# luicalrob/Triangulation-in-Deformable-Scenes

Measured on AMD Instinct MI355X. Metric: LM iterations/sec + ms/iter at 100k corr × 2 views; 1/2/4/8-GPU scaling, higher is better.
Workload: dtype f64

## Files before the change

### triangulation-in-deformable-scenes_amd/csrc/spcg.hip

```cpp
#include <hip/hip_runtime.h>

#include <algorithm>
#include <cstdio>
#include <type_traits>

#include "spcg.h"
#include "ticket.h"
#include "wave.h"

namespace deftri {
namespace sp {

using wv::wave_sum;
using wv::wave_max;

__device__ __forceinline__ double block_sum(double v, double *red4) {
    const int lane = threadIdx.x & 63, w = threadIdx.x >> 6;
    v = wave_sum(v);
    if (lane == 0) red4[w] = v;
    __syncthreads();
    const double s = (red4[0] + red4[1]) + (red4[2] + red4[3]);
    __syncthreads();
    return s;
}

__device__ __forceinline__ double pval(const double2 *__restrict__ zp, double beta, int64_t i) {
    const double2 v = zp[i];
    return __fma_rn(beta, v.y, v.x);
}

__device__ __forceinline__ int it_state(const SpDev &G, int it, double &beta) {
    beta = 0.0;
    if (G.rec[0] != 0.0) return (int)G.rec[0];
    const double *rk = G.red + (int64_t)kSpRed * it;
    if (rk[2] != 0.0) return (int)rk[2];
    if (rk[1] <= G.tol2 * G.red[1]) return kSpConverged;
    if (it >= G.max_it) return kSpBudget;
    if (it > 0) beta = rk[0] / G.red[(int64_t)kSpRed * (it - 1)];
    return 0;
}

__device__ __forceinline__ void record_stop(const SpDev &G, int it, int st) {
    if (G.rec[0] == 0.0) {
        G.rec[0] = st;
        G.rec[1] = it;
    }
}

__host__ __device__ __forceinline__ int row_grid(int nrb) { return 8 * ((max(nrb, 1) + 7) / 8); }
__device__ __forceinline__ int row_block(int b, int nrb) {
    const int seg = (max(nrb, 1) + 7) / 8;
    return (b & 7) * seg + (b >> 3);
}

__device__ __forceinline__ int heavy_dof(const SpDev &G, int h) { return h < G.Q ? 6 * h : 6 * G.Q + (h - G.Q); }

__device__ __forceinline__ bool gated_off(const int *g) { return g && !*g; }
__device__ __forceinline__ double lam_of(const SpDev &G, double lam) { return G.lam_dev ? *G.lam_dev : lam; }

__device__ __forceinline__ void publish(double *p, double v) { st_sc1(p, v); }
__device__ __forceinline__ double fetch(const double *p) {
    return ld_sc1(p);
}

__device__ __forceinline__ int tri3(int a, int b) { return a * (a + 1) / 2 + b; }
__device__ __forceinline__ int tri6(int a, int b) { return a * (a + 1) / 2 + b; }

template <class JT, int GU>
__global__ void __launch_bounds__(256) __attribute__((amdgpu_waves_per_eu(GU == 4 ? 5 : GU == 6 ? 4 : 1, GU == 4 ? 5 : GU == 6 ? 4 : 3)))
k_sp_glin_rows(const SpDev G, JT *__restrict__ pj) {
    __shared__ double red4[4];
    if (gated_off(G.lgate)) return;
    const int lb = row_block(blockIdx.x, G.nrb2);
    const int w = lb * 4 + (threadIdx.x >> 6), lane = threadIdx.x & 63;
    double mx = 0.0;
    if (w < G.nwaves) {
        const int l = G.rowmap[64 * w + lane];
        double D[6] = {0, 0, 0, 0, 0, 0}, bb[3] = {0, 0, 0};
        if (l >= 0) {
            for (int j = G.rep_off[l]; j < G.rep_off[l + 1]; j++) {
                const double *J = G.Jr + 6 * (int64_t)j;
                const double wt = G.Wr[j];
#pragma unroll
                for (int r = 0; r < 2; r++) {
                    const double er = G.Er[2 * (int64_t)j + r];
#pragma unroll
                    for (int a = 0; a < 3; a++) {
                        const double ja = J[3 * r + a] * wt;
#pragma unroll
                        for (int c = 0; c <= a; c++) D[tri3(a, c)] += ja * J[3 * r + c];
                        bb[a] -= J[3 * r + a] * (wt * er);
                    }
                }
            }
            const int d0 = G.dep_off[l], d1 = G.dep_off[l + 1];
            for (int jb = d0; jb < d1; jb += 4) {
                double Jb[4][4], wb[4], eb[4];
#pragma unroll
                for (int u = 0; u < 4; u++) {
                    const int64_t j = jb + u < d1 ? jb + u : jb;
#pragma unroll
                    for (int c = 0; c < 4; c++) Jb[u][c] = G.Jd[4 * j + c];
                    wb[u] = G.Wd[j];
                    eb[u] = G.Ed[j];
                }
#pragma unroll
                for (int u = 0; u < 4; u++) {
                    if (jb + u >= d1) break;
                    const int64_t j = jb + u;
                    const double *J = Jb[u];
                    const double wt = wb[u], er = eb[u];
#pragma unroll
                    for (int a = 0; a < 3; a++) {
                        const double ja = J[a] * wt;
#pragma unroll
                        for (int c = 0; c <= a; c++) D[tri3(a, c)] += ja * J[c];
                        bb[a] -= J[a] * (wt * er);
                        G.cdep[3 * j + a] = ja * J[3];
                    }
                    G.wss[j] = (J[3] * wt) * J[3];
                }
            }
        }
        double H[6];
#pragma unroll
        for (int k = 0; k < 6; k++) H[k] = D[k];
        const int64_t n = G.nslots * 64;
        struct Raw { double j0, j1, j2, w, x; };
        const double *__restrict__ Ja = G.Ja, *__restrict__ Wa = G.Wa, *__restrict__ Ea = G.Ea;
        const double *__restrict__ Jd = G.Jd, *__restrict__ Wd = G.Wd;
        const int64_t jld = G.jld;
        const bool w1 = G.Q == 1 && G.pinfo != nullptr;
        auto load = [&](int m) -> Raw {
            const bool dep = m <= -2;
            const int mm = max(m, 0), jj = max(-2 - m, 0);
            const double *pa = Ja + (int64_t)(3 * (mm & 3)) * jld + (mm >> 2);
            const double *pd = Jd + 4 * (int64_t)jj;
            const double *Jc = dep ? pd : pa;
            const int64_t st = dep ? 1 : jld;
            const double *W = dep ? Wd + jj : w1 ? G.pinfo : Wa + (mm >> 2);
            const double *X = dep ? pd + 3 : Ea + (mm >> 2);
            return Raw{Jc[0], Jc[st], Jc[2 * st], *W, *X};
        };
        auto value = [&](int m, const Raw &r, double *v, double &wt, double &er) {
            const bool arap = m >= 0, dep = m <= -2;
            v[0] = dep ? (r.j0 * r.w) * r.x : arap ? r.j0 : 0.0;
            v[1] = dep ? (r.j1 * r.w) * r.x : arap ? r.j1 : 0.0;
            v[2] = dep ? (r.j2 * r.w) * r.x : arap ? r.j2 : 0.0;
            wt = arap ? r.w : 0.0;
            er = arap ? r.x : 0.0;
        };
        auto add = [&](const double *v, double wt, double er) {
#pragma unroll
            for (int a = 0; a < 3; a++) {
                const double ja = v[a] * wt;
#pragma unroll
                for (int c = 0; c <= a; c++) H[tri3(a, c)] += ja * v[c];
                bb[a] -= v[a] * (wt * er);
            }
        };
        int64_t k = G.woff[w] * 64 + lane;
        const int64_t k1 = G.woff[w + 1] * 64 + lane;
        auto step = [&](auto U_, bool clamp) {
            constexpr int U = decltype(U_)::value;
            int m[U];
            int64_t kk[U];
            bool in[U];
            Raw r[U];
#pragma unroll
            for (int u = 0; u < U; u++) {
                in[u] = !clamp || k + 64 * u < k1;
                kk[u] = in[u] ? k + 64 * u : k1 - 64;
            }
#pragma unroll
            for (int u = 0; u < U; u++) m[u] = G.pmap[kk[u]];
#pragma unroll
            for (int u = 0; u < U; u++) r[u] = load(m[u]);
#pragma unroll
            for (int u = 0; u < U; u++) {
                double v[3], wt, er;
                value(m[u], r[u], v, wt, er);
                if (!in[u]) wt = er = 0.0;
                add(v, wt, er);
                if (pj)
#pragma unroll
                    for (int a = 0; a < 3; a++) pj[a * n + kk[u]] = (JT)v[a];
            }
            k += U * 64;
        };
        using I4 = std::integral_constant<int, 4>;
        if constexpr (GU == 4) {
            while (k + 3 * 64 < k1) step(I4{}, false);
        } else if constexpr (GU == 6) {
            while (k + 5 * 64 < k1) step(std::integral_constant<int, 6>{}, false);
            if (k + 4 * 64 < k1) step(std::integral_constant<int, 6>{}, true);
        } else {
            while (k + 7 * 64 < k1) step(std::integral_constant<int, 8>{}, false);
            if (k + 4 * 64 < k1) step(std::integral_constant<int, 8>{}, true);
        }
        if (k < k1) step(I4{}, true);
        if (G.wsplit[w]) {
#pragma unroll
            for (int k = 0; k < 6; k++) H[k] += __shfl_xor(H[k], 32);
#pragma unroll
            for (int a = 0; a < 3; a++) bb[a] += __shfl_xor(bb[a], 32);
        }
        if (l >= 0) {
#pragma unroll
            for (int k = 0; k < 6; k++) { G.Hv[6 * (int64_t)l + k] = H[k]; G.Dv[6 * (int64_t)l + k] = D[k]; }
            const int64_t o = G.hd + 3 * (int64_t)(G.row0 + l);
#pragma unroll
            for (int a = 0; a < 3; a++) G.b[o + a] = bb[a];
            mx = fmax(fabs(H[0]), fmax(fabs(H[2]), fabs(H[5])));
        }
    }
    mx = wave_max(mx);
    if ((threadIdx.x & 63) == 0) red4[threadIdx.x >> 6] = mx;
    __syncthreads();
    if (threadIdx.x == 0 && lb < max(G.nrb2, 1)) G.mpart[lb] = fmax(fmax(red4[0], red4[1]), fmax(red4[2], red4[3]));
}

__global__ void __launch_bounds__(256) k_sp_glin_blocks(const SpDev G) {
    __shared__ double red[kSpLin][4];
    if (gated_off(G.lgate)) return;
    const int2 gr = G.glb[blockIdx.x];
    const int4 d = G.blk[gr.x];
    const int kind = d.x & 0xff, owned = d.x >> 8;
    const int lane = threadIdx.x & 63, w = threadIdx.x >> 6;
    const int i = d.z + threadIdx.x;
    double *out = G.lpart + (int64_t)kSpLin * gr.x;
    if (kind == SP_ARAP) {
        if (!owned) return;
        double a[kSpLin];
#pragma unroll
        for (int k = 0; k < kSpLin; k++) a[k] = 0.0;
        const int iend = G.blk[gr.x + gr.y - 1].w;
        for (int ii = i; ii < iend; ii += 256) {
            double J[6];
#pragma unroll
            for (int r = 0; r < 6; r++) J[r] = G.Ja[(12 + r) * G.jld + ii];
            const double wv = G.Wa[ii], er = G.Ea[ii];
#pragma unroll
            for (int r = 0; r < 6; r++) {
                const double jr = J[r] * wv;
#pragma unroll
                for (int c = 0; c <= r; c++) a[tri6(r, c)] += jr * J[c];
                a[21 + r] -= J[r] * (wv * er);
            }
        }
        for (int k = threadIdx.x; k < kSpLin * (gr.y - 1); k += 256) out[kSpLin + k] = 0.0;
#pragma unroll
        for (int k = 0; k < kSpLin; k++) {
            const double v = wave_sum(a[k]);
            if (lane == 0) red[k][w] = v;
        }
        __syncthreads();
        if (threadIdx.x < kSpLin) {
            const int k = threadIdx.x;
            out[k] = (red[k][0] + red[k][1]) + (red[k][2] + red[k][3]);
        }
    } else {
        double h = 0.0, bs = 0.0;
        if (i < d.w) {
            const int le = G.dperm[i];
            const double js = G.Jd[4 * (int64_t)le + 3];
            h = G.wss[le];
            bs = -js * (G.Wd[le] * G.Ed[le]);
        }
        h = wave_sum(h);
        bs = wave_sum(bs);
        if (lane == 0) { red[0][w] = h; red[1][w] = bs; }
        __syncthreads();
        if (threadIdx.x < 2) {
            const int k = threadIdx.x;
            out[k] = (red[k][0] + red[k][1]) + (red[k][2] + red[k][3]);
        }
    }
}

__global__ void __launch_bounds__(256) k_sp_glin_heavy(const SpDev G) {
    __shared__ double lds[8][32];
    __shared__ int last;
    if (gated_off(G.lgate)) return;
    const int ch = blockIdx.x, h = G.ch_h[ch];
    const int dim = h < G.Q ? kSpLin : 2;
    const int c = threadIdx.x & 31, g = threadIdx.x >> 5;
    double acc = 0.0;
    if (c < dim) {
        int64_t k = G.ch_lo[ch] + g;
        const int64_t k1 = G.ch_lo[ch + 1];
        for (; k + 7 * 8 < k1; k += 64) {
            double v[8];
#pragma unroll
            for (int u = 0; u < 8; u++) v[u] = G.lpart[(int64_t)kSpLin * G.hv_blk[k + 8 * u] + c];
#pragma unroll
            for (int u = 0; u < 8; u++) acc += v[u];
        }
        for (; k < k1; k += 8) acc += G.lpart[(int64_t)kSpLin * G.hv_blk[k] + c];
    }
    lds[g][c] = acc;
    __syncthreads();
    if ((int)threadIdx.x < dim) {
        double t = 0.0;
#pragma unroll
        for (int gg = 0; gg < 8; gg++) t += lds[gg][threadIdx.x];
        publish(G.chpart + (int64_t)kSpLin * ch + threadIdx.x, t);
    }
    const int c0 = G.hch_off[h], c1 = G.hch_off[h + 1];
    if (threadIdx.x == 0) {
        __atomic_signal_fence(__ATOMIC_SEQ_CST);
        __builtin_amdgcn_s_waitcnt(0);
        __atomic_signal_fence(__ATOMIC_SEQ_CST);
        last = __hip_atomic_fetch_add(G.hcnt + h, 1, __ATOMIC_RELAXED, __HIP_MEMORY_SCOPE_AGENT) == c1 - c0 - 1;
    }
    __syncthreads();
    if (!last) return;
    acc = 0.0;
    if (c < dim)
        for (int j = c0 + g; j < c1; j += 8) acc += fetch(G.chpart + (int64_t)kSpLin * j + c);
    __syncthreads();
    lds[g][c] = acc;
    __syncthreads();
    if ((int)threadIdx.x < dim) {
        double t = 0.0;
#pragma unroll
        for (int gg = 0; gg < 8; gg++) t += lds[gg][threadIdx.x];
        const int q = threadIdx.x;
        if (h < G.Q) {
            if (q < 21) G.hl[21 * (int64_t)h + q] = t;
            else G.b[6 * (int64_t)h + q - 21] = t;
        } else {
            if (q == 0) G.hl[21 * (int64_t)G.Q + (h - G.Q)] = t;
            else G.b[6 * (int64_t)G.Q + (h - G.Q)] = t;
        }
    }
    if (threadIdx.x == 0) st_sc1(G.hcnt + h, 0);
}

__global__ void __launch_bounds__(256) k_sp_maxdiag(const SpDev G, double *out, int stage) {
    __shared__ double red4[4];
    if (gated_off(G.lgate)) return;
    double m = 0.0;
    if (stage == 0) {
        for (int i = threadIdx.x; i < G.nrb2; i += 256) m = fmax(m, G.mpart[i]);
    } else {
        for (int h = threadIdx.x; h < G.Q; h += 256)
#pragma unroll
            for (int a = 0; a < 6; a++) m = fmax(m, fabs(G.hl[21 * (int64_t)h + tri6(a, a)]));
        for (int s = threadIdx.x; s < G.S; s += 256) m = fmax(m, fabs(G.hl[21 * (int64_t)G.Q + s]));
    }
    m = wave_max(m);
    if ((threadIdx.x & 63) == 0) red4[threadIdx.x >> 6] = m;
    __syncthreads();
    if (threadIdx.x == 0) {
        const double v = fmax(fmax(red4[0], red4[1]), fmax(red4[2], red4[3]));
        out[0] = stage == 0 ? v : fmax(out[0], v);
    }
}

__global__ void k_sp_cvt_j(const double *__restrict__ J, float *__restrict__ J32, int64_t n, const int *gate) {
    if (gated_off(gate)) return;
    const int64_t i = (int64_t)blockIdx.x * 256 + threadIdx.x;
    if (i < n) J32[i] = (float)J[i];
}

__device__ __forceinline__ bool inv3(const double *A, double lam, double *M) {
    const double a00 = A[0] + lam, a10 = A[1], a11 = A[2] + lam, a20 = A[3], a21 = A[4], a22 = A[5] + lam;
    if (!(a00 > 0.0)) return false;
    const double l00 = sqrt(a00), l10 = a10 / l00, l20 = a20 / l00;
    const double d1 = a11 - l10 * l10;
    if (!(d1 > 0.0)) return false;
    const double l11 = sqrt(d1), l21 = (a21 - l20 * l10) / l11;
    const double d2 = a22 - l20 * l20 - l21 * l21;
    if (!(d2 > 0.0)) return false;
    const double l22 = sqrt(d2);
    const double i00 = 1.0 / l00, i11 = 1.0 / l11, i22 = 1.0 / l22;
    const double i10 = -l10 * i00 * i11;
    const double i21 = -l21 * i11 * i22;
    const double i20 = -(l20 * i00 + l21 * i10) * i22;
    M[0] = i00 * i00 + i10 * i10 + i20 * i20;
    M[1] = i11 * i10 + i21 * i20;
    M[2] = i11 * i11 + i21 * i21;
    M[3] = i22 * i20;
    M[4] = i22 * i21;
    M[5] = i22 * i22;
    return true;
}

__device__ __forceinline__ void mul3(const double *M, const double r[3], double z[3]) {
    z[0] = M[0] * r[0] + M[1] * r[1] + M[3] * r[2];
    z[1] = M[1] * r[0] + M[2] * r[1] + M[4] * r[2];
    z[2] = M[3] * r[0] + M[4] * r[1] + M[5] * r[2];
}

__device__ bool inv6(const double *Hl, double lam, double *Mo) {
    double L[36];
    for (int i = 0; i < 6; i++)
        for (int j = 0; j < 6; j++) L[i * 6 + j] = j <= i ? Hl[tri6(i, j)] + (i == j ? lam : 0.0) : 0.0;
    for (int j = 0; j < 6; j++) {
        double s = L[j * 6 + j];
        for (int k = 0; k < j; k++) s -= L[j * 6 + k] * L[j * 6 + k];
        if (!(s > 0.0)) return false;
        s = sqrt(s);
        L[j * 6 + j] = s;
        for (int i = j + 1; i < 6; i++) {
            double t = L[i * 6 + j];
            for (int k = 0; k < j; k++) t -= L[i * 6 + k] * L[j * 6 + k];
            L[i * 6 + j] = t / s;
        }
    }
    for (int c = 0; c < 6; c++) {
        double y[6];
        for (int i = 0; i < 6; i++) {
            double t = i == c ? 1.0 : 0.0;
            for (int k = 0; k < i; k++) t -= L[i * 6 + k] * y[k];
            y[i] = t / L[i * 6 + i];
        }
        for (int i = 5; i >= 0; i--) {
            double t = y[i];
            for (int k = i + 1; k < 6; k++) t -= L[k * 6 + i] * y[k];
            y[i] = t / L[i * 6 + i];
        }
        for (int i = 0; i < 6; i++) Mo[i * 6 + c] = y[i];
    }
    return true;
}

__device__ __forceinline__ void pair_tree(double a0, double a1, double (*red)[4], double *out, int pub = 0) {
    const int lane = threadIdx.x & 63, w = threadIdx.x >> 6;
    a0 = wave_sum(a0);
    a1 = wave_sum(a1);
    if (lane == 0) { red[0][w] = a0; red[1][w] = a1; }
    __syncthreads();
    if (threadIdx.x == 0) {
        const double s0 = (red[0][0] + red[0][1]) + (red[0][2] + red[0][3]);
        const double s1 = (red[1][0] + red[1][1]) + (red[1][2] + red[1][3]);
        if (pub == 1) {
            st_sc1(out, s0);
            st_sc1(out + 1, s1);
        } else {
            out[0] = s0;
            out[1] = s1;
        }
    }
}

__device__ __forceinline__ bool last_block(const SpDev &G, int *cnt) {
    __shared__ int last;
    if (threadIdx.x == 0) {
        __atomic_signal_fence(__ATOMIC_SEQ_CST);
        __builtin_amdgcn_s_waitcnt(0);
        __atomic_signal_fence(__ATOMIC_SEQ_CST);
        last = ticket_last(cnt, (int)gridDim.x, (int)blockIdx.x);
    }
    __syncthreads();
    return last;
}

template <int NV>
__device__ __forceinline__ bool group_sum(const SpDev &G, int *cnt, const double *slots, double *gs, double (*red)[4], double *tot) {
    __shared__ int flag;
    const int nb = (int)gridDim.x, x = (int)blockIdx.x & 7;
    const int gsize = (nb - x + 7) >> 3, ngroups = nb < 8 ? nb : 8;
    auto settle = [&] {
        __atomic_signal_fence(__ATOMIC_SEQ_CST);
        __builtin_amdgcn_s_waitcnt(0);
        __atomic_signal_fence(__ATOMIC_SEQ_CST);
    };
    if (threadIdx.x == 0) {
        settle();
        flag = __hip_atomic_fetch_add(cnt + 1 + x, 1, __ATOMIC_RELAXED, __HIP_MEMORY_SCOPE_AGENT) == gsize - 1;
    }
    __syncthreads();
    if (!flag) return false;
    double a[NV];
#pragma unroll
    for (int v = 0; v < NV; v++) a[v] = 0.0;
    for (int j = x + 8 * (int)threadIdx.x; j < nb; j += 8 * 256)
#pragma unroll
        for (int v = 0; v < NV; v++) a[v] += fetch(slots + NV * j + v);
    const int lane = threadIdx.x & 63, w = threadIdx.x >> 6;
#pragma unroll
    for (int v = 0; v < NV; v++) {
        a[v] = wave_sum(a[v]);
        if (lane == 0) red[v][w] = a[v];
    }
    __syncthreads();
    if (threadIdx.x == 0) {
#pragma unroll
        for (int v = 0; v < NV; v++) publish(gs + NV * x + v, (red[v][0] + red[v][1]) + (red[v][2] + red[v][3]));
        st_sc1(cnt + 1 + x, 0);
        settle();
        flag = __hip_atomic_fetch_add(cnt, 1, __ATOMIC_RELAXED, __HIP_MEMORY_SCOPE_AGENT) == ngroups - 1;
        if (flag) {
            st_sc1(cnt, 0);
#pragma unroll
            for (int v = 0; v < NV; v++) {
                double t = 0.0;
                for (int g = 0; g < ngroups; g++) t += fetch(gs + NV * g + v);
                tot[v] = t;
            }
        }
    }
    __syncthreads();
    return flag;
}

__device__ __forceinline__ void dots_block(const SpDev &G, int it, double (*red)[4]) {
    double a0 = 0.0, a1 = 0.0;
    int i = threadIdx.x;
    for (; i + 3 * 256 <= G.nrb; i += 4 * 256) {
        double v[4][2];
#pragma unroll
        for (int u = 0; u < 4; u++) { v[u][0] = fetch(G.upart + 2 * (i + 256 * u)); v[u][1] = fetch(G.upart + 2 * (i + 256 * u) + 1); }
#pragma unroll
        for (int u = 0; u < 4; u++) { a0 += v[u][0]; a1 += v[u][1]; }
    }
    for (; i <= G.nrb; i += 256) { a0 += fetch(G.upart + 2 * i); a1 += fetch(G.upart + 2 * i + 1); }
    pair_tree(a0, a1, red, G.red + (int64_t)kSpRed * it);
}

__device__ __forceinline__ void sd_send(const SpDev &G, int l, int a, double z, double p) {
    for (int k = G.snd_off[l]; k < G.snd_off[l + 1]; k++) {
        const int64_t o = 6 * (int64_t)G.snd_slot[k] + 2 * a;
        G.sbuf[o] = z;
        G.sbuf[o + 1] = p;
    }
}

__global__ void __launch_bounds__(3 * kSpUpdRows) k_sp_setup(const SpDev G, const double *__restrict__ rhs, double lam) {
    __shared__ double sM[6 * kSpUpdRows], sR[3 * kSpUpdRows];
    __shared__ double red[2][3 * kSpUpdRows / 64], dred[2][4];
    if (gated_off(G.gate)) return;
    lam = lam_of(G, lam);
    const int t = threadIdx.x, lane = t & 63, wv = t >> 6;
    constexpr int nw = 3 * kSpUpdRows / 64;
    double rz = 0.0, rr = 0.0;
    const int rb = (int)blockIdx.x - 1, slot = rb < 0 ? G.nrb : rb;
    if (rb < 0 && t < 32) st_sc1(G.cnt + t, 0);
    if (rb >= 0) {
        const int l0 = rb * kSpUpdRows;
        const int nrow = min(kSpUpdRows, G.nown - l0);
        const int64_t o0 = G.hd + 3 * (int64_t)(G.row0 + l0);
        const double *Hg = G.Hv + 6 * (int64_t)l0;
        if (t < 6 * nrow) sM[t] = Hg[t];
        if (t + 3 * kSpUpdRows < 6 * nrow) sM[t + 3 * kSpUpdRows] = Hg[t + 3 * kSpUpdRows];
        const double r = t < 3 * nrow ? rhs[o0 + t] : 0.0;
        sR[t] = r;
        __syncthreads();
        if (t < nrow) {
            double Hl[6], M[6];
#pragma unroll
            for (int k = 0; k < 6; k++) Hl[k] = sM[6 * t + k];
            if (!inv3(Hl, lam, M)) {
                G.rec[0] = kSpBadBlock;
#pragma unroll
                for (int k = 0; k < 6; k++) M[k] = 0.0;
            }
#pragma unroll
            for (int k = 0; k < 6; k++) sM[6 * t + k] = M[k];
        }
        __syncthreads();
        double *Mg = G.Mv + 6 * (int64_t)l0;
        if (t < 6 * nrow) Mg[t] = sM[t];
        if (t + 3 * kSpUpdRows < 6 * nrow) Mg[t + 3 * kSpUpdRows] = sM[t + 3 * kSpUpdRows];
        if (t < 3 * nrow) {
            const int row = t / 3, a = t - 3 * row;
            const double *M = sM + 6 * row;
            const int i0 = a == 0 ? 0 : a == 1 ? 1 : 3, i1 = a == 0 ? 1 : a == 1 ? 2 : 4, i2 = a == 0 ? 3 : a == 1 ? 4 : 5;
            const double *rv = sR + 3 * row;
            const double z = M[i0] * rv[0] + M[i1] * rv[1] + M[i2] * rv[2];
            G.r[o0 + t] = r;
            G.zp[o0 + t] = make_double2(z, 0.0);
            G.x[o0 + t] = 0.0;
            if (G.sd) sd_send(G, l0 + row, a, z, 0.0);
            rz = r * z;
            rr = r * r;
        }
    } else if (t < 256) {
        for (int h = t; h < G.Q + G.S; h += 256) {
// ... 1075 lines not shown
                    if (lane - d >= sstart) v[c] += y;
                }
            }
            if (valid && (m.x & kTmLast)) {
#pragma unroll
                for (int c = 0; c < 3; c++) { up[3 * ra + c] = v[c]; up[3 * rb + c] = v[3 + c]; }
            }
        }
        __syncthreads();
        if (tid < nr) {
            const int l = G.tmulti ? own_row(tid) : r0 + tid;
            const bool home = !G.tmulti || G.trow[r0 + tid] < 0;
            const int64_t o = G.hd + 3 * (int64_t)(G.row0 + l);
            double q[3], p[3];
#pragma unroll
            for (int c = 0; c < 3; c++) { q[c] = up[3 * tid + c]; p[c] = pL[3 * tid + c]; }
            const int sb = rsi & 0xffff, sc = rsi >> 16;
            for (int kk = sb; kk < sb + sc; kk++)
#pragma unroll
                for (int c = 0; c < 3; c++) q[c] += rs[3 * kk + c];
            if (home) {
                double D[6];
#pragma unroll
                for (int kk = 0; kk < 6; kk++) D[kk] = G.tmulti ? Dp[kk] : G.Dv[6 * (int64_t)l + kk];
                const double q0 = lam * p[0] + ((D[0] * p[0] + D[1] * p[1]) + D[3] * p[2]);
                const double q1 = lam * p[1] + ((D[1] * p[0] + D[2] * p[1]) + D[4] * p[2]);
                const double q2 = lam * p[2] + ((D[3] * p[0] + D[4] * p[1]) + D[5] * p[2]);
                pap += (p[0] * q0 + p[1] * q1) + p[2] * q2;
                q[0] += q0; q[1] += q1; q[2] += q2;
            }
            const int jend = G.tmulti ? (dsc0 >= 0 ? 1 : 0) : dj1 - dj0;
            for (int jj = 0; jj < jend; jj++) {
                const int j = dj0 + jj;
                const bool pre = G.tmulti != 0;
                const int sc_ = pre ? dsc0 : G.dsc[j];
                double cd[3];
#pragma unroll
                for (int c = 0; c < 3; c++) cd[c] = pre ? cd0[c] : G.cdep[3 * (int64_t)j + c];
                const double wsj = pre ? ws0 : G.wss[j];
                const double ps = hp[6 + sc_];
                const double cp = (cd[0] * p[0] + cd[1] * p[1]) + cd[2] * p[2];
                const double td = cp + wsj * ps;
                pap += ps * (cp + td);
                if (sc_ == 0) sacc[0] += td;
                else sacc[1] += td;
#pragma unroll
                for (int c = 0; c < 3; c++) q[c] += cd[c] * ps;
            }
            if (home) {
#pragma unroll
                for (int c = 0; c < 3; c++) G.q[o + c] = q[c];
            } else {
                const int64_t x = 3 * ((int64_t)(G.tdst[r0 + tid] - 1) * G.nown + l);
#pragma unroll
                for (int c = 0; c < 3; c++) G.qs[x + c] = q[c];
            }
        }
    }
    double a[9] = {pap, jts[0], jts[1], jts[2], jts[3], jts[4], jts[5], sacc[0], sacc[1]};
#pragma unroll
    for (int kk = 0; kk < 9; kk++) {
        const double v = wave_sum(a[kk]);
        if (lane == 0) red[kk][wv] = v;
    }
    __syncthreads();
    if (tid < 9) {
        const double v = (red[tid][0] + red[tid][1]) + (red[tid][2] + red[tid][3]);
        if (tid == 0) G.m1part[b] = v;
        else G.part[(int64_t)kSpPart * b + tid - 1] = v;
    }
}

template <int FIN>
__global__ void __launch_bounds__(256) k_sp_tupd(int it, const SpDev G, double lam, int last) {
    __shared__ double red4[4];
    if (gated_off(G.gate)) return;
    lam = lam_of(G, lam);
    double beta = 0.0;
    AlphaPre pf;
    const bool own_alpha = !FIN && !G.alpha_kernel && (G.tparts || blockIdx.x == 0);
    if (own_alpha) m2_alpha_loads(G, it, pf);
    if (const int st = it_state(G, it, beta)) {
        if (!FIN && blockIdx.x == 0 && threadIdx.x == 0) record_stop(G, it, st);
        return;
    }
    double alpha = 0.0, pq = 0.0, rr2 = 0.0;
    if (!FIN) {
        if (G.alpha_kernel) alpha = G.red[(int64_t)kSpRed * it + 3];
        else if (own_alpha) alpha = m2_alpha_make(G, it, red4, !G.tparts, pf, blockIdx.x == 0);
    }
    if ((int)blockIdx.x < G.m_nh) {
        __shared__ double lds[256];
        __shared__ double rsh[6], tz[2][6];
        const int h = blockIdx.x;
        const bool has = h < G.Q + G.S;
        const double th = has ? tile_heavy_sum(G, h, lds) : 0.0;
        if (!FIN && !own_alpha && !G.alpha_kernel) alpha = m2_alpha_wait(G, it);
        if (has) {
            const int dim = h < G.Q ? 6 : 1, o = heavy_dof(G, h);
            const int a = (!FIN && isnan(alpha)) ? dim : (int)threadIdx.x;
            double p = 0.0, r = 0.0;
            if (a < dim) {
                p = G.ph[o + a];
                const double q = th + lam * p;
                if (FIN) {
                    G.q[o + a] = q;
                } else {
                    G.x[o + a] += alpha * p;
                    r = G.r[o + a] - alpha * q;
                    G.r[o + a] = r;
                    rsh[a] = r;
                }
            }
            if (!FIN) {
                __syncthreads();
                if (a < dim) {
                    const double *Mh = h < G.Q ? G.Mh + 36 * (int64_t)h + a * 6 : G.Mh + 36 * (int64_t)G.Q + (h - G.Q);
                    double z = 0.0;
                    for (int c = 0; c < dim; c++) z += Mh[c] * rsh[c];
                    G.zp[o + a] = make_double2(z, p);
                    tz[0][a] = r * z;
                    tz[1][a] = r * r;
                }
                __syncthreads();
                if (threadIdx.x == 0 && !isnan(alpha))
                    for (int c = 0; c < dim; c++) { pq += tz[0][c]; rr2 += tz[1][c]; }
            }
        }
    } else {
        const int lb = row_block((int)blockIdx.x - G.m_nh, G.nrb);
        const int l = lb * 256 + (int)threadIdx.x;
        const bool on = l < G.nown;
        double q[3] = {0, 0, 0}, pr[3] = {0, 0, 0}, xo[3] = {0, 0, 0}, ro[3] = {0, 0, 0}, M[6] = {0, 0, 0, 0, 0, 0};
        int64_t o = 0;
        if (on) {
            o = G.hd + 3 * (int64_t)l;
#pragma unroll
            for (int c = 0; c < 3; c++) q[c] = G.q[o + c];
            if (G.tmulti) {
                const int ns = G.tnshare[l];
                for (int j0 = 1; j0 < ns; j0 += 4) {
                    double v[4][3];
#pragma unroll
                    for (int u = 0; u < 4; u++) {
                        const int j = j0 + u < ns ? j0 + u : j0;
                        const double *s = G.qs + 3 * ((int64_t)(j - 1) * G.nown + l);
#pragma unroll
                        for (int c = 0; c < 3; c++) v[u][c] = s[c];
                    }
#pragma unroll
                    for (int u = 0; u < 4; u++)
                        if (j0 + u < ns)
#pragma unroll
                            for (int c = 0; c < 3; c++) q[c] += v[u][c];
                }
            }
            {
                const int k0 = G.txoff[l], k1 = G.txoff[l + 1];
                for (int kb = k0; kb < k1; kb += 4) {
                    double v[4][3];
#pragma unroll
                    for (int u = 0; u < 4; u++) {
                        const int64_t k = kb + u < k1 ? kb + u : kb;
#pragma unroll
                        for (int c = 0; c < 3; c++) v[u][c] = G.xc[3 * k + c];
                    }
#pragma unroll
                    for (int u = 0; u < 4; u++)
                        if (kb + u < k1)
#pragma unroll
                            for (int c = 0; c < 3; c++) q[c] += v[u][c];
                }
            }
            if (FIN) {
#pragma unroll
                for (int c = 0; c < 3; c++) G.q[o + c] = q[c];
            } else {
#pragma unroll
                for (int c = 0; c < 3; c++) {
                    const double2 v = G.zp[o + c];
                    pr[c] = __fma_rn(beta, v.y, v.x);
                    xo[c] = G.x[o + c];
                    ro[c] = G.r[o + c];
                }
#pragma unroll
                for (int k = 0; k < 6; k++) M[k] = G.Mv[6 * (int64_t)l + k];
            }
        }
        if (!FIN && !own_alpha && !G.alpha_kernel) alpha = m2_alpha_wait(G, it);
        if (!FIN && on && !isnan(alpha)) {
            double r[3], z[3];
#pragma unroll
            for (int c = 0; c < 3; c++) {
                G.x[o + c] = xo[c] + alpha * pr[c];
                r[c] = ro[c] - alpha * q[c];
            }
            z[0] = M[0] * r[0] + M[1] * r[1] + M[3] * r[2];
            z[1] = M[1] * r[0] + M[2] * r[1] + M[4] * r[2];
            z[2] = M[3] * r[0] + M[4] * r[1] + M[5] * r[2];
#pragma unroll
            for (int c = 0; c < 3; c++) {
                G.r[o + c] = r[c];
                G.zp[o + c] = make_double2(z[c], pr[c]);
                pq += r[c] * z[c];
                rr2 += r[c] * r[c];
            }
        }
    }
    if (FIN) return;
    __shared__ double red[2][4];
    if (G.tparts && !last) {
        pair_tree(pq, rr2, red, G.m2part + 2 * blockIdx.x, 0);
        return;
    }
    pair_tree(pq, rr2, red, G.m2part + 2 * blockIdx.x, 1);
    m2_dots(G, it, red);
}

__global__ void __launch_bounds__(256) k_sp_txb(int it, const SpDev G) {
    __shared__ double red4[4];
    __shared__ double lds[256];
    (void)it;
    if (gated_off(G.gate) || G.rec[0] != 0.0) return;
    const int nh = G.Q + G.S, h = (int)blockIdx.x;
    if (h < nh) {
        const double t = tile_heavy_sum(G, h, lds);
        if ((int)threadIdx.x < (h < G.Q ? 6 : 1)) G.xb[3 + heavy_dof(G, h) + threadIdx.x] = t;
    } else if (h == nh) {
        double a = 0.0;
        for (int j = threadIdx.x; j < G.t_grid; j += 256) a += G.m1part[j];
        a = block_sum(a, red4);
        if (threadIdx.x == 0) G.xb[2] = a;
    } else {
        double a0 = 0.0, a1 = 0.0;
        for (int j = threadIdx.x; j <= G.nrb; j += 256) { a0 += G.upart[2 * j]; a1 += G.upart[2 * j + 1]; }
        a0 = block_sum(a0, red4);
        a1 = block_sum(a1, red4);
        if (threadIdx.x == 0) { G.xb[0] = a0; G.xb[1] = a1; }
    }
}


__global__ void k_sp_pack(int n, const int32_t *__restrict__ rows, int width, int64_t base, const double *__restrict__ src,
                          double *__restrict__ buf) {
    const int64_t t = (int64_t)blockIdx.x * 256 + threadIdx.x;
    if (t >= (int64_t)n * width) return;
    const int64_t i = t / width, c = t % width;
    buf[t] = src[base + (int64_t)width * rows[i] + c];
}

__global__ void k_sp_unpack(int n, const int32_t *__restrict__ rows, int width, int64_t base, const double *__restrict__ buf,
                            double *__restrict__ dst) {
    const int64_t t = (int64_t)blockIdx.x * 256 + threadIdx.x;
    if (t >= (int64_t)n * width) return;
    const int64_t i = t / width, c = t % width;
    dst[base + (int64_t)width * rows[i] + c] = buf[t];
}

__global__ void k_sp_load_p(int64_t n, const double *__restrict__ v, double2 *__restrict__ zp) {
    const int64_t t = (int64_t)blockIdx.x * 256 + threadIdx.x;
    if (t < n) zp[t] = make_double2(v[t], 0.0);
}

__global__ void k_sp_permute(int32_t P, int64_t hd, const int32_t *__restrict__ row_of_point, const double *__restrict__ src,
                             double *__restrict__ dst, int to_plan) {
    const int64_t t = (int64_t)blockIdx.x * 256 + threadIdx.x;
    if (t < hd) { dst[t] = src[t]; return; }
    const int64_t u = t - hd;
    if (u >= 3 * (int64_t)P) return;
    const int64_t pt = u / 3, c = u % 3;
    const int64_t row = row_of_point[pt];
    if (to_plan) dst[hd + 3 * row + c] = src[hd + 3 * pt + c];
    else dst[hd + 3 * pt + c] = src[hd + 3 * row + c];
}

}

static inline unsigned nblk(int64_t n, int bs) { return (unsigned)std::max<int64_t>((n + bs - 1) / bs, 1); }

#define SPL(NAME, KER, GRID, ...)                                          \
    do {                                                                   \
        if ((GRID) <= 0) break;                               \
        hipEvent_t e0_ = prof_begin(st);                                   \
        hipLaunchKernelGGL(KER, dim3(GRID), dim3(256), 0, st, __VA_ARGS__); \
        prof_end(NAME, e0_, (unsigned)(GRID), 0.0, st);                    \
    } while (0)

#define SPLS(NAME, KER, GRID, LDS, ...)                                              \
    do {                                                                             \
        if ((GRID) <= 0) break;                                                      \
        hipEvent_t e0_ = prof_begin(st);                                             \
        hipLaunchKernelGGL(KER, dim3(GRID), dim3(256), (size_t)(LDS), st, __VA_ARGS__); \
        prof_end(NAME, e0_, (unsigned)(GRID), 0.0, st);                              \
    } while (0)

template <class JT, int MG>
static void launch_phase2(const SpDev &G, int grid, int it, double lambda, const JT *pj, hipStream_t st) {
    if (G.p2u == 4) SPL("sp_phase2", (sp::k_sp_phase2<JT, MG, 4>), grid, it, G, lambda, pj);
    else if (G.p2u == 6) SPL("sp_phase2", (sp::k_sp_phase2<JT, MG, 6>), grid, it, G, lambda, pj);
    else SPL("sp_phase2", (sp::k_sp_phase2<JT, MG, 8>), grid, it, G, lambda, pj);
}

void sp_launch_glin(const SpDev &G, bool fp32, hipStream_t st) {
    if (G.glu == 4) {
        if (fp32) SPL("sp_glin_rows", (sp::k_sp_glin_rows<float, 4>), sp::row_grid(G.nrb2), G, G.pj32);
        else SPL("sp_glin_rows", (sp::k_sp_glin_rows<double, 4>), sp::row_grid(G.nrb2), G, G.pj);
    } else if (G.glu == 6) {
        if (fp32) SPL("sp_glin_rows", (sp::k_sp_glin_rows<float, 6>), sp::row_grid(G.nrb2), G, G.pj32);
        else SPL("sp_glin_rows", (sp::k_sp_glin_rows<double, 6>), sp::row_grid(G.nrb2), G, G.pj);
    } else {
        if (fp32) SPL("sp_glin_rows", (sp::k_sp_glin_rows<float, 8>), sp::row_grid(G.nrb2), G, G.pj32);
        else SPL("sp_glin_rows", (sp::k_sp_glin_rows<double, 8>), sp::row_grid(G.nrb2), G, G.pj);
    }
    if (G.nblk > 0) SPL("sp_glin_blocks", sp::k_sp_glin_blocks, G.nglb, G);
    if (G.nch > 0) SPL("sp_glin_heavy", sp::k_sp_glin_heavy, G.nch, G);
}

void sp_launch_maxdiag(const SpDev &G, double *out, hipStream_t st) {
    SPL("sp_maxdiag", sp::k_sp_maxdiag, 1, G, out, 0);
}

void sp_launch_maxdiag_heavy(const SpDev &G, double *out, hipStream_t st) {
    SPL("sp_maxdiag", sp::k_sp_maxdiag, 1, G, out, 1);
}

void sp_launch_cvt_j(const double *J, float *J32, int64_t n, hipStream_t st, const int *gate) {
    if (n > 0) SPL("sp_cvt_j", sp::k_sp_cvt_j, nblk(n, 256), J, J32, n, gate);
}

void sp_launch_setup(const SpDev &G, const double *rhs, double lambda, hipStream_t st) {
    const int grid = (G.nown + kSpUpdRows - 1) / kSpUpdRows + 1;
    hipEvent_t e0_ = prof_begin(st);
    hipLaunchKernelGGL(sp::k_sp_setup, dim3(grid), dim3(3 * kSpUpdRows), 0, st, G, rhs, lambda);
    prof_end("sp_setup", e0_, (unsigned)grid, 0.0, st);
}

void sp_launch_dots(const SpDev &G, int it, hipStream_t st) {
    SPL("sp_dots", sp::k_sp_dots, 1, it, G);
}

void sp_launch_product(const SpDev &G, int it, double lambda, bool fp32, hipStream_t st, bool last) {
    if (G.sd) {
        sp_launch_sd_phase1(G, it, lambda, fp32, st, nullptr, sp_merged_grid1(G));
        sp_launch_sd_phase2(G, it, lambda, fp32, st);
        return;
    }
    if (G.tile) {
        hipEvent_t e0_ = prof_begin(st);
        if (fp32) hipLaunchKernelGGL((sp::k_sp_tile<float>), dim3(G.t_grid), dim3(256), (size_t)G.tile_lds, st, it, G, G.Ja32, lambda);
        else hipLaunchKernelGGL((sp::k_sp_tile<double>), dim3(G.t_grid), dim3(256), (size_t)G.tile_lds, st, it, G, G.Ja, lambda);
        prof_end("sp_tile", e0_, (unsigned)G.t_grid, 0.0, st);
        if (G.alpha_kernel) SPL("sp_alpha", sp::k_sp_alpha, 1, it, G);
        SPL("sp_tupd", (sp::k_sp_tupd<0>), G.m_nh + sp::row_grid(G.nrb), it, G, lambda, last ? 1 : 0);
        return;
    }
    if (G.merged) {
        const int g1 = sp_merged_grid1(G), g2 = sp_merged_grid2(G);
        if (fp32) SPL("sp_phase1", (sp::k_sp_phase1<float, 1>), g1, it, G, G.Ja32, lambda);
        else SPL("sp_phase1", (sp::k_sp_phase1<double, 1>), g1, it, G, G.Ja, lambda);
        if (G.alpha_kernel) SPL("sp_alpha", sp::k_sp_alpha, 1, it, G);
        if (fp32) launch_phase2<float, 1>(G, g2, it, lambda, G.pj32, st);
        else launch_phase2<double, 1>(G, g2, it, lambda, G.pj, st);
        return;
    }
    if (G.nblk > 0) {
        if (fp32) SPL("sp_phase1", (sp::k_sp_phase1<float, 0>), G.nblk, it, G, G.Ja32, lambda);
        else SPL("sp_phase1", (sp::k_sp_phase1<double, 0>), G.nblk, it, G, G.Ja, lambda);
    }
    const int grid = sp::row_grid(G.nrb2) + (G.fuse_heavy ? G.Q + G.S : 0);
    if (fp32) launch_phase2<float, 0>(G, grid, it, lambda, G.pj32, st);
    else launch_phase2<double, 0>(G, grid, it, lambda, G.pj, st);
}

void sp_launch_tile_sd(const SpDev &G, int it, double lambda, bool fp32, hipStream_t st, const int32_t *list, int n,
                       bool txb) {
    if (n > 0) {
        SpDev g = G;
        g.p1list = list;
        hipEvent_t e0_ = prof_begin(st);
        if (fp32) hipLaunchKernelGGL((sp::k_sp_tile<float, 1>), dim3(n), dim3(256), (size_t)G.tile_lds, st, it, g, G.Ja32, lambda);
        else hipLaunchKernelGGL((sp::k_sp_tile<double, 1>), dim3(n), dim3(256), (size_t)G.tile_lds, st, it, g, G.Ja, lambda);
        prof_end("sp_tile", e0_, (unsigned)n, 0.0, st);
    }
    if (txb) SPL("sp_txb", sp::k_sp_txb, G.Q + G.S + 2, it, G);
}

void sp_launch_tile_product(const SpDev &G, double lambda, bool fp32, hipStream_t st) {
    hipEvent_t e0_ = prof_begin(st);
    if (fp32) hipLaunchKernelGGL((sp::k_sp_tile<float>), dim3(G.t_grid), dim3(256), (size_t)G.tile_lds, st, 0, G, G.Ja32, lambda);
    else hipLaunchKernelGGL((sp::k_sp_tile<double>), dim3(G.t_grid), dim3(256), (size_t)G.tile_lds, st, 0, G, G.Ja, lambda);
    prof_end("sp_tile", e0_, (unsigned)G.t_grid, 0.0, st);
    SPL("sp_tupd", (sp::k_sp_tupd<1>), G.m_nh + sp::row_grid(G.nrb), 0, G, lambda, 1);
}

int sp_merged_grid1(const SpDev &G) { return 8 * ((G.nrb + 1 + 7) / 8) + G.nblk; }

void sp_launch_sd_phase1(const SpDev &G, int it, double lambda, bool fp32, hipStream_t st, const int32_t *list, int n) {
    SpDev g = G;
    g.p1list = list;
    if (fp32) SPL("sp_phase1", (sp::k_sp_phase1<float, 2>), n, it, g, G.Ja32, lambda);
    else SPL("sp_phase1", (sp::k_sp_phase1<double, 2>), n, it, g, G.Ja, lambda);
}

void sp_launch_sd_phase2(const SpDev &G, int it, double lambda, bool fp32, hipStream_t st) {
    const int g2 = G.m_nh + sp::row_grid(G.nrb2);
    if (fp32) launch_phase2<float, 2>(G, g2, it, lambda, G.pj32, st);
    else launch_phase2<double, 2>(G, g2, it, lambda, G.pj, st);
}
int sp_merged_grid2(const SpDev &G) { return 8 * ((G.Q + G.S + 7) / 8) + sp::row_grid(G.nrb2); }

void sp_launch_heavy(const SpDev &G, int it, double lambda, int stage, hipStream_t st) {
    const int grid = (stage == 1 && G.heavy_split) ? G.Q + G.S + 1 : 1;
    SPL("sp_heavy", sp::k_sp_heavy, grid, it, G, lambda, stage);
}

void sp_launch_update_sd(const SpDev &G, int it, double lambda, int tail, hipStream_t st) {
    const int grid = (G.nown + kSpUpdRows - 1) / kSpUpdRows + 1;
    hipEvent_t e0_ = prof_begin(st);
    hipLaunchKernelGGL(sp::k_sp_update_sd, dim3(grid), dim3(3 * kSpUpdRows), 0, st, it, G, lambda, tail);
    prof_end("sp_update", e0_, (unsigned)grid, 0.0, st);
}

void sp_launch_update(const SpDev &G, int it, hipStream_t st) {
    const int grid = (G.nown + kSpUpdRows - 1) / kSpUpdRows + 1;
    hipEvent_t e0_ = prof_begin(st);
    hipLaunchKernelGGL(sp::k_sp_update, dim3(grid), dim3(3 * kSpUpdRows), 0, st, it, G);
    prof_end("sp_update", e0_, (unsigned)grid, 0.0, st);
}

void sp_launch_halo_pack(int n, const int32_t *rows, int width, int64_t base, const double *src, double *buf,
                         hipStream_t st) {
    if (n > 0) SPL("sp_halo_pack", sp::k_sp_pack, nblk((int64_t)n * width, 256), n, rows, width, base, src, buf);
}

void sp_launch_halo_unpack(int n, const int32_t *rows, int width, int64_t base, const double *buf, double *dst,
                           hipStream_t st) {
    if (n > 0) SPL("sp_halo_unpack", sp::k_sp_unpack, nblk((int64_t)n * width, 256), n, rows, width, base, buf, dst);
}

void sp_launch_load_p(int64_t n, const double *v, double2 *zp, hipStream_t st) {
    SPL("sp_load_p", sp::k_sp_load_p, nblk(n, 256), n, v, zp);
}

void sp_launch_permute_in(int32_t P, int64_t hd, const int32_t *row_of_point, const double *src, double *dst,
                          hipStream_t st) {
    SPL("sp_permute", sp::k_sp_permute, nblk(hd + 3 * (int64_t)P, 256), P, hd, row_of_point, src, dst, 1);
}

void sp_launch_permute_out(int32_t P, int64_t hd, const int32_t *row_of_point, const double *src, double *dst,
                           hipStream_t st) {
    SPL("sp_permute", sp::k_sp_permute, nblk(hd + 3 * (int64_t)P, 256), P, hd, row_of_point, src, dst, 0);
}

}
```

Baseline: 1742.

## Fuse glin row and block kernels into one launch with batched ARAP loads

Merges the row-wise and block-wise linearization kernels into a single kernel that branches on block index, removing one launch and letting both kinds of work share the GPU at once. The ARAP accumulation loop now loads T items' Jacobians ahead before doing the FMAs, to raise memory-level parallelism. The data-term Hessian is recomputed from Jd and Wd instead of reading a precomputed wss array. In exchange, the block path now runs under the row kernel's waves-per-eu occupancy attribute and needs more registers for the prefetch buffers.

```diff
diff --git a/triangulation-in-deformable-scenes_amd/csrc/spcg.hip b/triangulation-in-deformable-scenes_amd/csrc/spcg.hip
--- a/triangulation-in-deformable-scenes_amd/csrc/spcg.hip
+++ b/triangulation-in-deformable-scenes_amd/csrc/spcg.hip
@@ -67,10 +67,7 @@
 __device__ __forceinline__ int tri6(int a, int b) { return a * (a + 1) / 2 + b; }
 
 template <class JT, int GU>
-__global__ void __launch_bounds__(256) __attribute__((amdgpu_waves_per_eu(GU == 4 ? 5 : GU == 6 ? 4 : 1, GU == 4 ? 5 : GU == 6 ? 4 : 3)))
-k_sp_glin_rows(const SpDev G, JT *__restrict__ pj) {
-    __shared__ double red4[4];
-    if (gated_off(G.lgate)) return;
+__device__ __forceinline__ void glin_rows(const SpDev &G, JT *__restrict__ pj, double *red4) {
     const int lb = row_block(blockIdx.x, G.nrb2);
     const int w = lb * 4 + (threadIdx.x >> 6), lane = threadIdx.x & 63;
     double mx = 0.0;
@@ -220,10 +217,9 @@
     if (threadIdx.x == 0 && lb < max(G.nrb2, 1)) G.mpart[lb] = fmax(fmax(red4[0], red4[1]), fmax(red4[2], red4[3]));
 }
 
-__global__ void __launch_bounds__(256) k_sp_glin_blocks(const SpDev G) {
-    __shared__ double red[kSpLin][4];
-    if (gated_off(G.lgate)) return;
-    const int2 gr = G.glb[blockIdx.x];
+template <int T>
+__device__ __forceinline__ void glin_blocks(const SpDev &G, int b, double (*red)[4]) {
+    const int2 gr = G.glb[b];
     const int4 d = G.blk[gr.x];
     const int kind = d.x & 0xff, owned = d.x >> 8;
     const int lane = threadIdx.x & 63, w = threadIdx.x >> 6;
@@ -235,17 +231,28 @@
 #pragma unroll
         for (int k = 0; k < kSpLin; k++) a[k] = 0.0;
         const int iend = G.blk[gr.x + gr.y - 1].w;
-        for (int ii = i; ii < iend; ii += 256) {
-            double J[6];
-#pragma unroll
-            for (int r = 0; r < 6; r++) J[r] = G.Ja[(12 + r) * G.jld + ii];
-            const double wv = G.Wa[ii], er = G.Ea[ii];
-#pragma unroll
-            for (int r = 0; r < 6; r++) {
-                const double jr = J[r] * wv;
-#pragma unroll
-                for (int c = 0; c <= r; c++) a[tri6(r, c)] += jr * J[c];
-                a[21 + r] -= J[r] * (wv * er);
+        for (int ii = i; ii < iend; ii += 256 * T) {
+            double Jb[T][6], wb[T], eb[T];
+#pragma unroll
+            for (int u = 0; u < T; u++) {
+                const int iu = ii + 256 * u < iend ? ii + 256 * u : ii;
+#pragma unroll
+                for (int r = 0; r < 6; r++) Jb[u][r] = G.Ja[(12 + r) * G.jld + iu];
+                wb[u] = G.Wa[iu];
+                eb[u] = G.Ea[iu];
+            }
+#pragma unroll
+            for (int u = 0; u < T; u++) {
+                if (ii + 256 * u >= iend) break;
+                const double *J = Jb[u];
+                const double wv = wb[u], er = eb[u];
+#pragma unroll
+                for (int r = 0; r < 6; r++) {
+                    const double jr = J[r] * wv;
+#pragma unroll
+                    for (int c = 0; c <= r; c++) a[tri6(r, c)] += jr * J[c];
+                    a[21 + r] -= J[r] * (wv * er);
+                }
             }
         }
         for (int k = threadIdx.x; k < kSpLin * (gr.y - 1); k += 256) out[kSpLin + k] = 0.0;
@@ -263,9 +270,9 @@
         double h = 0.0, bs = 0.0;
         if (i < d.w) {
             const int le = G.dperm[i];
-            const double js = G.Jd[4 * (int64_t)le + 3];
-            h = G.wss[le];
-            bs = -js * (G.Wd[le] * G.Ed[le]);
+            const double js = G.Jd[4 * (int64_t)le + 3], wt = G.Wd[le];
+            h = (js * wt) * js;
+            bs = -js * (wt * G.Ed[le]);
         }
         h = wave_sum(h);
         bs = wave_sum(bs);
@@ -276,6 +283,15 @@
             out[k] = (red[k][0] + red[k][1]) + (red[k][2] + red[k][3]);
         }
     }
+}
+
+template <class JT, int GU>
+__global__ void __launch_bounds__(256) __attribute__((amdgpu_waves_per_eu(GU == 4 ? 5 : GU == 6 ? 4 : 1, GU == 4 ? 5 : GU == 6 ? 4 : 3)))
+k_sp_glin(const SpDev G, JT *__restrict__ pj, int nrows) {
+    __shared__ double red[kSpLin][4];
+    if (gated_off(G.lgate)) return;
+    if ((int)blockIdx.x < nrows) glin_rows<JT, GU>(G, pj, red[0]);
+    else glin_blocks<GU == 8 ? 4 : 2>(G, blockIdx.x - nrows, red);
 }
 
 __global__ void __launch_bounds__(256) k_sp_glin_heavy(const SpDev G) {
@@ -1957,17 +1973,17 @@
 }
 
 void sp_launch_glin(const SpDev &G, bool fp32, hipStream_t st) {
+    const int nrows = sp::row_grid(G.nrb2), grid = nrows + (G.nblk > 0 ? G.nglb : 0);
     if (G.glu == 4) {
-        if (fp32) SPL("sp_glin_rows", (sp::k_sp_glin_rows<float, 4>), sp::row_grid(G.nrb2), G, G.pj32);
-        else SPL("sp_glin_rows", (sp::k_sp_glin_rows<double, 4>), sp::row_grid(G.nrb2), G, G.pj);
+        if (fp32) SPL("sp_glin_rows", (sp::k_sp_glin<float, 4>), grid, G, G.pj32, nrows);
+        else SPL("sp_glin_rows", (sp::k_sp_glin<double, 4>), grid, G, G.pj, nrows);
     } else if (G.glu == 6) {
-        if (fp32) SPL("sp_glin_rows", (sp::k_sp_glin_rows<float, 6>), sp::row_grid(G.nrb2), G, G.pj32);
-        else SPL("sp_glin_rows", (sp::k_sp_glin_rows<double, 6>), sp::row_grid(G.nrb2), G, G.pj);
+        if (fp32) SPL("sp_glin_rows", (sp::k_sp_glin<float, 6>), grid, G, G.pj32, nrows);
+        else SPL("sp_glin_rows", (sp::k_sp_glin<double, 6>), grid, G, G.pj, nrows);
     } else {
-        if (fp32) SPL("sp_glin_rows", (sp::k_sp_glin_rows<float, 8>), sp::row_grid(G.nrb2), G, G.pj32);
-        else SPL("sp_glin_rows", (sp::k_sp_glin_rows<double, 8>), sp::row_grid(G.nrb2), G, G.pj);
-    }
-    if (G.nblk > 0) SPL("sp_glin_blocks", sp::k_sp_glin_blocks, G.nglb, G);
+        if (fp32) SPL("sp_glin_rows", (sp::k_sp_glin<float, 8>), grid, G, G.pj32, nrows);
+        else SPL("sp_glin_rows", (sp::k_sp_glin<double, 8>), grid, G, G.pj, nrows);
+    }
     if (G.nch > 0) SPL("sp_glin_heavy", sp::k_sp_glin_heavy, G.nch, G);
 }
 
```

After: 1773, median of 6. 1.8% higher.
